# madronalabs/madronalib

Hardware: AMD Instinct MI355X
Metric: voice-samples/sec (SawGen->SVF chain) (higher is better)
Workload: dtype f32

## Files before the change

### madronalib_amd/csrc/mldsp_kernels.hpp

```cpp
#pragma once
#include "mlgpu_device_args.hpp"
#include "mldsp_procs.hpp"

namespace mldev
{
typedef float f32x4 __attribute__((ext_vector_type(4)));

constexpr int kChainBlock = 256;

constexpr int kMixStrip = 64 * 20 + 3 * 16 + 16;
template <int LO, int N>
struct MixTree16
{
  static __device__ __forceinline__ float sum(const float* col) { return MixTree16<LO, N / 2>::sum(col) + MixTree16<LO + N / 2, N / 2>::sum(col); }
};
template <int LO>
struct MixTree16<LO, 1>
{
  static __device__ __forceinline__ float sum(const float* col) { return col[LO * 20]; }
};

__device__ __forceinline__ void mix64_park(float* strip, int qq, f32x4 y)
{
  const uint32_t lane = threadIdx.x & 63u;
  *(f32x4*)(strip + lane * 20 + (lane >> 4) * 16 + 4 * qq) = y;
}
__device__ __forceinline__ void mix64_sum_store(const float* strip, float* row16)
{
  const uint32_t lane = threadIdx.x & 63u;
  __builtin_amdgcn_fence(__ATOMIC_RELEASE, "wavefront");
  __builtin_amdgcn_wave_barrier();
  __builtin_amdgcn_fence(__ATOMIC_ACQUIRE, "wavefront");
  const uint32_t s = lane & 15u, g = lane >> 4;
  const float t16 = MixTree16<0, 16>::sum(strip + g * (16 * 20 + 16) + s);
  const float t32 = t16 + u2f((uint32_t)__builtin_amdgcn_ds_bpermute((int)(((lane + 16u) & 63u) * 4u), (int)f2u(t16)));
  const float t64 = t32 + u2f((uint32_t)__builtin_amdgcn_ds_bpermute((int)(((lane + 32u) & 63u) * 4u), (int)f2u(t32)));
  if (lane < 16) row16[s] = t64;
  __builtin_amdgcn_wave_barrier();
}

template <bool MIX>
struct MixStrips
{
  static __device__ __forceinline__ float* mine() { return nullptr; }
};
template <>
struct MixStrips<true>
{
  static __device__ __forceinline__ float* mine()
  {
    __shared__ __attribute__((aligned(16))) float lds[(256 / 64) * kMixStrip];
    return lds + (threadIdx.x >> 6) * kMixStrip;
  }
};

constexpr int kHeadGeneral = 0, kHeadFast = 1, kHeadTrip = 2;
constexpr int kHeadTripSamples = 8;

template <class CH, bool HAS_SIGNAL, int HEAD, bool MIX = false, bool SCALED = false, bool LISTED = false>
__device__ __forceinline__ void run_voice(CH& ch, const ChainArgs& a, size_t v, float xc, float* strip = nullptr, bool live = true, size_t vs = 0,
                                          uint32_t* peak = nullptr)
{
  static_assert(HEAD != kHeadTrip || (!HAS_SIGNAL && CH::kHeadHasTrip), "trips want a launch-constant input and a head that has them");
  const size_t vin = LISTED ? vs : v;
  uint32_t pk = 0;
  const float mixGain = (SCALED && a.mixGains) ? a.mixGains[vin] : 1.f;
  const f32x4* pin = HAS_SIGNAL ? (const f32x4*)a.in.base + vin * a.in.strideV : nullptr;
  f32x4* pout = MIX ? nullptr : (f32x4*)a.out.base + v * a.out.strideV;
  const size_t inQ = a.in.strideQ, outQ = a.out.strideQ;
  const uint32_t slot = wave_slot();
  for (size_t t = 0; t < a.T; ++t)
  {
    const f32x4* pi = HAS_SIGNAL ? pin + t * a.in.strideT : nullptr;
    f32x4* po = MIX ? nullptr : pout + t * a.out.strideT;
    float s[kHeadTripSamples];
#pragma unroll 4
    for (int q = 0; q < 16; ++q)
    {
      if ((q & 3) == 0) take_turns_by_clock(slot, kTurnClockShift);
      f32x4 y;
      if constexpr (HEAD == kHeadTrip)
      {
        static_assert(kHeadTripSamples == 8, "a trip is two quads");
        if ((q & 1) == 0) ch.template next_head_trip<kHeadTripSamples>(xc, s);
        y = (q & 1) ? f32x4{s[4], s[5], s[6], s[7]} : f32x4{s[0], s[1], s[2], s[3]};
      }
      else
      {
        f32x4 x = {xc, xc, xc, xc};
        if constexpr (HAS_SIGNAL) x = __builtin_nontemporal_load(pi + q * inQ);
        y.x = ch.template next_head<HEAD == kHeadFast>(x.x);
        y.y = ch.template next_head<HEAD == kHeadFast>(x.y);
        y.z = ch.template next_head<HEAD == kHeadFast>(x.z);
        y.w = ch.template next_head<HEAD == kHeadFast>(x.w);
      }
      if constexpr (LISTED)
      {
        const uint32_t m0 = f2u(y.x) & 0x7fffffffu, m1 = f2u(y.y) & 0x7fffffffu, m2 = f2u(y.z) & 0x7fffffffu, m3 = f2u(y.w) & 0x7fffffffu;
        const uint32_t m01 = m0 > m1 ? m0 : m1, m23 = m2 > m3 ? m2 : m3, m = m01 > m23 ? m01 : m23;
        pk = pk > m ? pk : m;
      }
      if constexpr (MIX)
      {
        if constexpr (SCALED)
        {
          if (a.mixGains)
          {
            y.x *= mixGain;
            y.y *= mixGain;
            y.z *= mixGain;
            y.w *= mixGain;
          }
          if (!live) y = f32x4{0.f, 0.f, 0.f, 0.f};
        }
        mix64_park(strip, q & 3, y);
        if ((q & 3) == 3) mix64_sum_store(strip, a.mix + ((v >> 6) * a.T + t) * 64 + (size_t)(q & ~3) * 4);
      }
      else
        __builtin_nontemporal_store(y, po + q * outQ);
    }
    ch.end_vector();
  }
  if constexpr (LISTED) *peak = pk;
}

template <class CH, bool HAS_SIGNAL, bool MIX, bool SCALED, bool LISTED>
__device__ __forceinline__ void run_voice_as(int head, CH& ch, const ChainArgs& a, size_t v, float xc, float* strip, bool live, size_t vs, uint32_t* peak)
{
  if constexpr (!HAS_SIGNAL && CH::kHeadHasTrip)
  {
    if (head == kHeadTrip)
    {
      run_voice<CH, HAS_SIGNAL, kHeadTrip, MIX, SCALED, LISTED>(ch, a, v, xc, strip, live, vs, peak);
      return;
    }
  }
  if (head != kHeadGeneral)
    run_voice<CH, HAS_SIGNAL, kHeadFast, MIX, SCALED, LISTED>(ch, a, v, xc, strip, live, vs, peak);
  else
    run_voice<CH, HAS_SIGNAL, kHeadGeneral, MIX, SCALED, LISTED>(ch, a, v, xc, strip, live, vs, peak);
}

template <int OUT_G>
struct GroupStrips
{
  static __device__ __forceinline__ float* mine() { return nullptr; }
};
template <>
struct GroupStrips<16>
{
  static __device__ __forceinline__ float* mine()
  {
    __shared__ __attribute__((aligned(16))) float lds[(256 / 64) * kGroup16Strip];
    return lds + (threadIdx.x >> 6) * kGroup16Strip;
  }
};

template <class CH, bool HAS_SIGNAL, bool FAST_HEAD, int OUT_G, bool GAINS>
__device__ __forceinline__ void run_voice_groups(CH& ch, const ChainArgs& a, size_t v, float xc, float* strip)
{
  static_assert(OUT_G == 1 || OUT_G == 2 || OUT_G == 4 || OUT_G == 8 || OUT_G == 16, "group_sum_in_order's sizes, or none");
  const float gain = GAINS ? a.mixGains[v] : 1.f;
  const f32x4* pin = HAS_SIGNAL ? (const f32x4*)a.in.base + (v >> a.inGroupShift) * a.in.strideV : nullptr;
  f32x4* pout = (f32x4*)a.out.base + (v / OUT_G) * a.out.strideV;
  const bool lastOfGroup = (threadIdx.x & (OUT_G - 1)) == OUT_G - 1;
  const size_t inQ = a.in.strideQ, outQ = a.out.strideQ;
  const uint32_t slot = wave_slot();
  for (size_t t = 0; t < a.T; ++t)
  {
    const f32x4* pi = HAS_SIGNAL ? pin + t * a.in.strideT : nullptr;
    f32x4* po = pout + t * a.out.strideT;
#pragma unroll 4
    for (int q = 0; q < 16; ++q)
    {
      if ((q & 3) == 0) take_turns_by_clock(slot, kTurnClockShift);
      f32x4 x = {xc, xc, xc, xc};
      if constexpr (HAS_SIGNAL) x = __builtin_nontemporal_load(pi + q * inQ);
      f32x4 y;
      y.x = ch.template next_head<FAST_HEAD>(x.x);
      y.y = ch.template next_head<FAST_HEAD>(x.y);
      y.z = ch.template next_head<FAST_HEAD>(x.z);
      y.w = ch.template next_head<FAST_HEAD>(x.w);
      if constexpr (GAINS)
      {
        y.x *= gain;
        y.y *= gain;
        y.z *= gain;
        y.w *= gain;
      }
      if constexpr (OUT_G == 1)
        __builtin_nontemporal_store(y, po + q * outQ);
      else if constexpr (OUT_G == 16)
      {
        group16_park(strip, q & 3, y);
        if ((q & 3) == 3) group16_sum_store(strip, po + (size_t)(q - 3) * outQ, outQ);
      }
      else
      {
        y.x = group_sum_in_order<OUT_G>(y.x);
        y.y = group_sum_in_order<OUT_G>(y.y);
        y.z = group_sum_in_order<OUT_G>(y.z);
        y.w = group_sum_in_order<OUT_G>(y.w);
        if (lastOfGroup) __builtin_nontemporal_store(y, po + q * outQ);
      }
    }
    ch.end_vector();
  }
}

template <class CH, bool HAS_SIGNAL, bool MIX = false, int OUT_G = 0, bool LISTED = false>
__device__ __forceinline__ void chain_kernel_body(const ChainArgs& a)
{
  static_assert(!(MIX && OUT_G), "one summing form at a time");
  static_assert(!(LISTED && OUT_G), "no group form of a voice list");
  apply_fp_mode(a.flags);
  __shared__ float ldsTable[CH::kHasImpulse ? 32 : 1];
  float* const strip = OUT_G ? GroupStrips<OUT_G>::mine() : MixStrips<MIX>::mine();
  if constexpr (CH::kHasImpulse)
  {
    if (threadIdx.x < Proc<MLGPU_PROC_IMPULSE_GEN>::kTableSize) ldsTable[threadIdx.x] = a.impulseTable[threadIdx.x];
    __syncthreads();
  }
  size_t blk = blockIdx.x;
  const size_t nbFull = (size_t)gridDim.x & ~(size_t)7;
  if (blk < nbFull) blk = (blk & 7) * (nbFull >> 3) + (blk >> 3);
  size_t v = blk * kChainBlock + threadIdx.x;
  bool live = true;
  if constexpr (MIX)
  {
    if ((v & ~(size_t)63) >= a.V) return;
    live = v < a.V;
    if (!live) v = a.V - 1;
  }
  else if (v >= a.V)
    return;

  size_t vs = v, stride = a.V;
  if constexpr (LISTED)
  {
    vs = a.voiceList[v];
    stride = a.tableStride;
  }
  uint32_t pk = 0;

  CH ch;
  const VoiceMem mem{a.coeffs + vs, a.state + vs, stride};
  const KernelTables tables{ldsTable};
  ch.load(mem, tables);

  const float xc = (!HAS_SIGNAL && a.inConst) ? a.inConst[vs] : 0.f;

  bool fastHead = false;
  if constexpr (!HAS_SIGNAL && CH::kHeadHasFastPath) fastHead = (__builtin_amdgcn_ballot_w64(CH::head_input_is_odd(xc)) == 0);
  int head = fastHead ? kHeadFast : kHeadGeneral;
  if constexpr (!HAS_SIGNAL && CH::kHeadHasTrip)
  {
    if (fastHead && __builtin_amdgcn_ballot_w64(trip_freq_is_dense(xc, kHeadTripSamples)) == 0) head = kHeadTrip;
  }
  if constexpr (OUT_G != 0)
  {
    if (a.mixGains != nullptr)
    {
      if (fastHead)
        run_voice_groups<CH, HAS_SIGNAL, true, OUT_G, true>(ch, a, v, xc, strip);
      else
        run_voice_groups<CH, HAS_SIGNAL, false, OUT_G, true>(ch, a, v, xc, strip);
    }
    else if (fastHead)
      run_voice_groups<CH, HAS_SIGNAL, true, OUT_G, false>(ch, a, v, xc, strip);
    else
      run_voice_groups<CH, HAS_SIGNAL, false, OUT_G, false>(ch, a, v, xc, strip);
  }
  else if constexpr (MIX)
  {
    const bool scaled = a.mixGains != nullptr || __builtin_amdgcn_ballot_w64(!live) != 0;
    if (scaled)
      run_voice_as<CH, HAS_SIGNAL, true, true, LISTED>(head, ch, a, v, xc, strip, live, vs, &pk);
    else
      run_voice_as<CH, HAS_SIGNAL, true, false, LISTED>(head, ch, a, v, xc, strip, live, vs, &pk);
  }
  else
    run_voice_as<CH, HAS_SIGNAL, false, false, LISTED>(head, ch, a, v, xc, strip, live, vs, &pk);
  ch.store(mem);
  if constexpr (LISTED)
  {
    if (a.peaks != nullptr)
    {
      if (live) a.peaks[v] = pk;
    }
  }
}

template <class CH, bool HAS_SIGNAL>
__global__ __launch_bounds__(kChainBlock) void chain_kernel(const ChainArgs a)
{
  chain_kernel_body<CH, HAS_SIGNAL>(a);
}

template <class CH, bool HAS_SIGNAL>
__global__ __launch_bounds__(kChainBlock) void chain_mix_kernel(const ChainArgs a)
{
  chain_kernel_body<CH, HAS_SIGNAL, true>(a);
}

template <class CH, bool HAS_SIGNAL>
__global__ __launch_bounds__(kChainBlock) void chain_listed_kernel(const ChainArgs a)
{
  chain_kernel_body<CH, HAS_SIGNAL, false, 0, true>(a);
}
template <class CH, bool HAS_SIGNAL>
__global__ __launch_bounds__(kChainBlock) void chain_listed_mix_kernel(const ChainArgs a)
{
  chain_kernel_body<CH, HAS_SIGNAL, true, 0, true>(a);
}

template <class CH, bool HAS_SIGNAL, int OUT_G>
__global__ __launch_bounds__(kChainBlock) void chain_group_kernel(const ChainArgs a)
{
  chain_kernel_body<CH, HAS_SIGNAL, false, OUT_G>(a);
}

typedef float f32x2 __attribute__((ext_vector_type(2)));

template <int KIND, int N>
struct SvfCascade
{
  static_assert(N % 2 == 0, "stages are evaluated in pairs");
  static constexpr int NCK = (KIND == MLGPU_PROC_HIPASS) ? 4 : 3;
  static constexpr int NC = NCK * N, NS = 2 * N;
  static constexpr int H = N / 2;
  f32x2 g0[H], g1[H], g2[H], kk[H], ic1[H], ic2[H], r[H];

  template <class ARR>
  static MLD void put(ARR& arr, int s, float value)
  {
    if (s < H)
      arr[s].x = value;
    else
      arr[s - H].y = value;
  }
  template <class ARR>
  static MLD float get(const ARR& arr, int s) { return s < H ? arr[s].x : arr[s - H].y; }

  MLD void load(const VoiceMem& m)
  {
#pragma unroll
    for (int s = 0; s < N; ++s)
    {
      put(g0, s, m.c(NCK * s));
      put(g1, s, m.c(NCK * s + 1));
      put(g2, s, m.c(NCK * s + 2));
      put(kk, s, (KIND == MLGPU_PROC_HIPASS) ? m.c(NCK * s + 3) : 0.f);
      put(ic1, s, u2f(m.s(2 * s)));
      put(ic2, s, u2f(m.s(2 * s + 1)));
      put(r, s, 0.f);
    }
  }
  MLD void store(const VoiceMem& m) const
  {
#pragma unroll
    for (int s = 0; s < N; ++s)
    {
      m.set(2 * s, f2u(get(ic1, s)));
      m.set(2 * s + 1, f2u(get(ic2, s)));
    }
  }
  MLD float tick(float x) { return tick_in0(f32x2{x, r[H - 1].x}); }
  MLD float tick_in0(f32x2 in0) { return tick_common<false>(in0, in0); }
  MLD float tick_t0(f32x2 t00)
  {
    static_assert(KIND != MLGPU_PROC_HIPASS, "Hipass reads its input twice");
    return tick_common<true>(t00, t00);
  }
  template <bool HAVE_T0>
  MLD float tick_common(f32x2 in0, f32x2 t00)
  {
    f32x2 in[H], t0[H], a[H], b[H], c[H], d[H], t1[H], t2[H], v1[H], v2[H];
    const f32x2 two = {2.0f, 2.0f};
    in[0] = in0;
#pragma unroll
    for (int p = 1; p < H; ++p) in[p] = r[p - 1];
#pragma unroll
    for (int p = 0; p < H; ++p) t0[p] = in[p] - ic2[p];
    if constexpr (HAVE_T0) t0[0] = t00;
#pragma unroll
    for (int p = 0; p < H; ++p) b[p] = g1[p] * ic1[p];
#pragma unroll
    for (int p = 0; p < H; ++p) d[p] = g0[p] * ic1[p];
#pragma unroll
    for (int p = 0; p < H; ++p) a[p] = g0[p] * t0[p];
#pragma unroll
    for (int p = 0; p < H; ++p) c[p] = g2[p] * t0[p];
#pragma unroll
    for (int p = 0; p < H; ++p) t1[p] = a[p] + b[p];
#pragma unroll
    for (int p = 0; p < H; ++p) t2[p] = c[p] + d[p];
    if (KIND == MLGPU_PROC_LOPASS)
    {
#pragma unroll
      for (int p = 0; p < H; ++p) r[p] = t2[p] + ic2[p];
    }
    else if (KIND == MLGPU_PROC_BANDPASS)
    {
#pragma unroll
      for (int p = 0; p < H; ++p) r[p] = t1[p] + ic1[p];
    }
    else
    {
#pragma unroll
      for (int p = 0; p < H; ++p) v1[p] = t1[p] + ic1[p];
#pragma unroll
      for (int p = 0; p < H; ++p) v2[p] = t2[p] + ic2[p];
#pragma unroll
      for (int p = 0; p < H; ++p) v1[p] = kk[p] * v1[p];
#pragma unroll
      for (int p = 0; p < H; ++p) v1[p] = in[p] - v1[p];
#pragma unroll
      for (int p = 0; p < H; ++p) r[p] = v1[p] - v2[p];
    }
#pragma unroll
    for (int p = 0; p < H; ++p) ic1[p] = MLGPU_SVF_STRICT ? ic1[p] + two * t1[p] : __builtin_elementwise_fma(two, t1[p], ic1[p]);
#pragma unroll
    for (int p = 0; p < H; ++p) ic2[p] = MLGPU_SVF_STRICT ? ic2[p] + two * t2[p] : __builtin_elementwise_fma(two, t2[p], ic2[p]);
    return r[H - 1].y;
  }
  MLD float tick_masked(float x, int sLo, int sHi)
  {
    float in[N];
    in[0] = x;
#pragma unroll
    for (int s = 1; s < N; ++s) in[s] = get(r, s - 1);
#pragma unroll
    for (int s = 0; s < N; ++s)
    {
      if (s >= sLo && s <= sHi)
      {
        const float i1 = get(ic1, s), i2 = get(ic2, s);
        const float t0 = in[s] - i2;
        const float t1 = get(g0, s) * t0 + get(g1, s) * i1;
        const float t2 = get(g2, s) * t0 + get(g0, s) * i1;
        if (KIND == MLGPU_PROC_LOPASS)
          put(r, s, t2 + i2);
        else if (KIND == MLGPU_PROC_BANDPASS)
          put(r, s, t1 + i1);
        else
          put(r, s, in[s] - get(kk, s) * (t1 + i1) - (t2 + i2));
        put(ic1, s, svf_acc(i1, t1));
        put(ic2, s, svf_acc(i2, t2));
      }
    }
    return get(r, N - 1);
  }
};

template <class HEAD, int KIND, int N, bool HAS_SIGNAL>
__global__ __launch_bounds__(kChainBlock) void cascade_kernel(const ChainArgs a)
{
  static_assert(!HEAD::kHasImpulse, "ImpulseGen heads are not supported by the cascade kernel");
  static_assert((N - 1) % 4 != 0, "cascade lengths with (N - 1) % 4 == 0 need a bounded prefetch");
  apply_fp_mode(a.flags);
  size_t blk = blockIdx.x;
  const size_t nbFull = (size_t)gridDim.x & ~(size_t)7;
  if (blk < nbFull) blk = (blk & 7) * (nbFull >> 3) + (blk >> 3);
  const size_t v = blk * kChainBlock + threadIdx.x;
  if (v >= a.V) return;

  HEAD head;
  SvfCascade<KIND, N> c;
  const VoiceMem mh{a.coeffs + v, a.state + v, a.V};
  const VoiceMem mc{a.coeffs + (size_t)HEAD::NC * a.V + v, a.state + (size_t)HEAD::NS * a.V + v, a.V};
  const KernelTables tables{nullptr};
  head.load(mh, tables);
  c.load(mc);
  const float xc = (!HAS_SIGNAL && a.inConst) ? a.inConst[v] : 0.f;

  constexpr int D = N - 1;
  constexpr int A = D / 4, B = D % 4;
  const size_t S = a.T * 64;
  const f32x4* pin = HAS_SIGNAL ? (const f32x4*)a.in.base + v * a.in.strideV : nullptr;
  f32x4* pout = (f32x4*)a.out.base + v * a.out.strideV;
  auto inQuad = [&](size_t qi) { return pin + (qi >> 4) * a.in.strideT + (qi & 15) * a.in.strideQ; };
  auto outQuad = [&](size_t qi) { return pout + (qi >> 4) * a.out.strideT + (qi & 15) * a.out.strideQ; };
  auto inAt = [&](size_t i) -> float {
    if constexpr (HAS_SIGNAL) return ((const float*)inQuad(i >> 2))[i & 3];
    return xc;
  };

  for (int i = 0; i < D; ++i) c.tick_masked(head.next(inAt((size_t)i)), 0, i);

  constexpr int QT = 4;
  const size_t Q = (S - D) / 4;
  size_t q = 0;
  if constexpr (HAS_SIGNAL)
  {
    f32x4 w[QT + 1];
    if (Q >= QT)
    {
#pragma unroll
      for (int k = 0; k < QT + 1; ++k) w[k] = __builtin_nontemporal_load(inQuad((size_t)(A + k)));
    }
    for (; q + QT <= Q; q += QT)
    {
      const bool more = (q + 2 * QT <= Q);
      f32x4 nx[QT];
      if (more)
      {
#pragma unroll
        for (int k = 0; k < QT; ++k) nx[k] = __builtin_nontemporal_load(inQuad(q + A + QT + 1 + k));
      }
#pragma unroll
      for (int g = 0; g < QT; ++g)
      {
        f32x4 y;
#pragma unroll
        for (int j = 0; j < 4; ++j)
        {
          const int e = B + j;
          const float x = (e < 4) ? w[g][e & 3] : w[g + 1][e & 3];
          y[j] = c.tick(head.next(x));
        }
        __builtin_nontemporal_store(y, outQuad(q + g));
      }
      if (more)
      {
        w[0] = w[QT];
#pragma unroll
        for (int k = 0; k < QT; ++k) w[k + 1] = nx[k];
      }
    }
  }
  else
  {
    for (; q + 4 <= Q; q += 4)
    {
#pragma unroll
      for (int g = 0; g < 4; ++g)
      {
        f32x4 y;
#pragma unroll
        for (int j = 0; j < 4; ++j) y[j] = c.tick(head.next(xc));
        __builtin_nontemporal_store(y, outQuad(q + g));
      }
    }
  }
  for (size_t i = D + 4 * q; i < S + D; ++i)
  {
    float x = 0.f;
    if (i < S) x = head.next(inAt(i));
    const int sLo = (i < S) ? 0 : (int)(i - S + 1);
    const float y = c.tick_masked(x, sLo, N - 1);
    const size_t n = i - D;
    ((float*)outQuad(n >> 2))[n & 3] = y;
  }
  head.store(mh);
  c.store(mc);
}

template <int LPC>
struct LaneGroup
{
// ... 150 lines not shown
```

### madronalib_amd/csrc/mldsp_procs.hpp

```cpp
#pragma once
#include "mldsp_math.hpp"
#ifdef __HIPCC_RTC__
#include "mlgpu.h"
#else
#include "../../include/mlgpu.h"
#endif

namespace mldev
{
struct VoiceMem
{
  const float* coeffs;
  uint32_t* state;
  size_t V;
  float* mem{nullptr};
  uint32_t memMask{0};
  MLD float* ringPtr(int ringIdx, uint32_t i) const
  {
    if (addr32) return (float*)((char*)(mem + (size_t)((uint32_t)ringIdx * (memMask + 1)) * V) + (__umul24(i, V4) + lane4));
    return mem + (size_t)((uint32_t)ringIdx * (memMask + 1) + i) * V;
  }
  MLD float ring(int ringIdx, uint32_t i) const { return *ringPtr(ringIdx, i); }
  MLD void ringSet(int ringIdx, uint32_t i, float x) const { *ringPtr(ringIdx, i) = x; }
  float* lds{nullptr};
  uint32_t ldsHist{0};
  uint32_t lane4{0}, V4{0};
  bool addr32{false};
  MLD float c(int i) const { return coeffs[(size_t)i * V]; }
  MLD uint32_t s(int i) const { return state[(size_t)i * V]; }
  MLD void set(int i, uint32_t x) const { state[(size_t)i * V] = x; }
};

struct KernelTables
{
  const float* impulse_table;
};

constexpr float kStepsPerCycle = 4294967296.0f;
constexpr float kCyclesPerStep = 2.3283064365386963e-10f;

constexpr uint32_t kSqrt2Bits = 0x3fb50505u;
constexpr uint32_t kSineDomainBits = 0x40b50505u;
constexpr uint32_t kSineScaleBits = 0x3f87c3b6u;
constexpr uint32_t kSineFlipBits = 0x40350505u;
constexpr uint32_t kOneSixthBits = 0x3e2aaaabu;

MLD float phasor_next(uint32_t& omega32, float cyclesPerSample)
{
  const float steps = cyclesPerSample * kStepsPerCycle;
  const int32_t istep = sse_cvt(steps);
  omega32 += (uint32_t)istep;
  const float hi = (float)(int32_t)(omega32 >> 1);
  return hi * 4.656612873077392578125e-10f;
}

constexpr float kPhaseUnit = 4.656612873077392578125e-10f;
constexpr float kPhaseScale = 2147483648.0f;
MLD float phasor_next_hi(uint32_t& omega32, float cyclesPerSample)
{
  const float steps = cyclesPerSample * kStepsPerCycle;
  const int32_t istep = sse_cvt(steps);
  omega32 += (uint32_t)istep;
  asm("" : "+v"(omega32));
  return (float)(int32_t)(omega32 >> 1);
}

MLD float div_nr(float n, float d)
{
  const float r0 = __builtin_amdgcn_rcpf(d);
  const float e = __builtin_fmaf(-d, r0, 1.0f);
  const float r1 = __builtin_fmaf(e, r0, r0);
  const float q0 = n * r1;
  const float rem0 = __builtin_fmaf(-d, q0, n);
  const float q1 = __builtin_fmaf(rem0, r1, q0);
  const float rem1 = __builtin_fmaf(-d, q1, n);
  return __builtin_fmaf(rem1, r1, q1);
}

MLD bool blep_freq_is_odd(float dt) { return (dt > 0.f) && !((dt >= 0x1p-64f) && (dt <= 0x1p+64f)); }

MLD bool blep_freq_not_regular(float dt) { return (f2u(dt) - 0x1F800000u) > (0x5F800000u - 0x1F800000u); }

template <bool FAST>
struct BlepFreq
{
  float dt, omdt;
  bool otherOdd;
  static MLD BlepFreq make(float dt, bool otherwiseOdd = false)
  {
    BlepFreq f;
    f.dt = dt;
    f.omdt = 1.0f - dt;
    f.otherOdd = otherwiseOdd;
    return f;
  }
  MLD bool lo(float t) const { return t < dt; }
  MLD bool hi(float t) const { return t > omdt; }
  MLD bool anyLaneOdd() const { return __builtin_amdgcn_ballot_w64((!FAST && blep_freq_not_regular(dt)) || otherOdd) != 0; }
  MLD float correction(float t, bool isLo, bool full) const
  {
    const float num = isLo ? t : (t - 1.0f);
    float q;
    if (full)
      q = num / dt;
    else
      q = div_nr(num, dt);
    const float qq = q * q;
    const float twoq_qq = full ? ((q + q) - qq) : __builtin_fmaf(2.0f, q, -qq);
    const float clo = twoq_qq - 1.0f;
    const float chi = ((qq + q) + q) + 1.0f;
    return isLo ? clo : chi;
  }
};

template <bool SKIP, bool FAST>
MLD float poly_blep(float t, const BlepFreq<FAST>& f)
{
  const bool lo = f.lo(t), hi = f.hi(t);
  if (SKIP && __builtin_amdgcn_ballot_w64(lo || hi) == 0) return 0.f;
  const float c = f.correction(t, lo, f.anyLaneOdd());
  return (lo || hi) ? c : 0.f;
}
template <bool FAST, bool SKIP = false>
MLD float poly_blep(float t, float dt)
{
  return poly_blep<SKIP>(t, BlepFreq<FAST>::make(dt));
}

MLD bool phase_is_odd(float p) { return !(((p >= 0x1p-31f) && (p <= 1.0f)) || (p == 0.f)); }

template <bool FAST, bool SKIP = false, bool ANY_PHASE = false>
MLD float phasor_to_saw(float p, float cps)
{
  const float saw = ANY_PHASE ? (p * 2.f - 1.f) : __builtin_fmaf(p, 2.f, -1.f);
  return saw - poly_blep<SKIP>(p, BlepFreq<FAST>::make(cps, ANY_PHASE && phase_is_odd(p)));
}

MLD bool pulse_width_is_odd(float w) { return !(w >= 0.f && w <= 1.0f); }

template <bool FAST, bool SKIP = false, bool ANY_PHASE = false, bool REGULAR_W = false>
MLD float phasor_to_pulse(float p, float cps, float w)
{
  const float pulse = (p >= w) ? -1.f : 1.f;
  const float d = p - w + 1.0f;
  const float down = REGULAR_W ? __builtin_amdgcn_fractf(d) : d - (float)sse_cvtt(d);
  const bool downOdd = ANY_PHASE ? phase_is_odd(down) : (!REGULAR_W && !(abs_ps(down) <= 2.0f));
  const BlepFreq<FAST> f = BlepFreq<FAST>::make(cps, (ANY_PHASE && phase_is_odd(p)) || downOdd);
  const bool loUp = f.lo(p), nearUp = loUp || f.hi(p);
  const bool loDown = f.lo(down), nearDown = loDown || f.hi(down);
  if (SKIP && __builtin_amdgcn_ballot_w64(nearUp || nearDown) == 0) return pulse;
  const bool full = f.anyLaneOdd();
  if (!(ANY_PHASE && full) && __builtin_amdgcn_ballot_w64(nearUp && nearDown) == 0)
  {
    const float c = f.correction(nearDown ? down : p, nearDown ? loDown : loUp, full);
    return nearDown ? (pulse - c) : (nearUp ? (pulse + c) : pulse);
  }
  const float cUp = f.correction(p, loUp, full), cDown = f.correction(down, loDown, full);
  return (pulse + (nearUp ? cUp : 0.f)) - (nearDown ? cDown : 0.f);
}

constexpr float kTripMaxFreq(int n) { return 0.5f / (float)n; }
constexpr float kTripTiny = 0x1p-22f, kTripNearOne = 1.0f - 0x1p-22f;
constexpr float kTripTinyShifted = 0x1p-21f, kTripNearOneShifted = 1.0f - 0x1p-21f;
MLD bool trip_freq_is_dense(float dt, int n) { return !(dt > 0.f && dt <= kTripMaxFreq(n)); }
MLD uint32_t trip_umin(uint32_t a, uint32_t b) { return a < b ? a : b; }
MLD uint32_t trip_umax(uint32_t a, uint32_t b) { return a > b ? a : b; }

MLD float phasor_to_sine(float p)
{
  const float sqrt2 = u2f(kSqrt2Bits);
  const float omega = p * u2f(kSineDomainBits) + (-sqrt2);
  const float tri = (omega > sqrt2) ? (u2f(kSineFlipBits) - omega) : omega;
  return (u2f(kSineScaleBits) * tri) * (1.0f - (tri * tri) * u2f(kOneSixthBits));
}

MLD float phasor_hi_to_sine(float hi)
{
  const float sqrt2 = u2f(kSqrt2Bits);
  const float omega = hi * u2f(kSineDomainBits - (31u << 23)) + (-sqrt2);
  const float refl = u2f(kSineFlipBits) - omega;
  float tri;
  asm("v_min_f32 %0, %1, %2" : "=v"(tri) : "v"(omega), "v"(refl));
  return (u2f(kSineScaleBits) * tri) * (1.0f - (tri * tri) * u2f(kOneSixthBits));
}

template <int KIND>
struct Proc;


template <>
struct Proc<MLGPU_PROC_PHASOR_GEN>
{
  static constexpr int NC = 0, NS = 1;
  uint32_t omega32;
  MLD void load(const VoiceMem& m, const KernelTables&) { omega32 = m.s(0); }
  MLD void store(const VoiceMem& m) const { m.set(0, omega32); }
  MLD float next(float cps) { return phasor_next(omega32, cps); }
  MLD void end_vector() {}
};

template <>
struct Proc<MLGPU_PROC_SINE_GEN>
{
  static constexpr int NC = 0, NS = 1;
  uint32_t omega32;
  MLD void load(const VoiceMem& m, const KernelTables&) { omega32 = m.s(0); }
  MLD void store(const VoiceMem& m) const { m.set(0, omega32); }
  MLD float next(float cps) { return phasor_hi_to_sine(phasor_next_hi(omega32, cps)); }
  MLD void end_vector() {}
};

template <>
struct Proc<MLGPU_PROC_TEST_SINE_GEN>
{
  static constexpr int NC = 0, NS = 1;
  float omega;
  MLD void load(const VoiceMem& m, const KernelTables&) { omega = u2f(m.s(0)); }
  MLD void store(const VoiceMem& m) const { m.set(0, f2u(omega)); }
  MLD float next(float cps)
  {
    const float twoPi = 6.2831853071795864769252867f;
    const float step = twoPi * cps;
    omega += step;
    if (omega > twoPi) omega -= twoPi;
    return libm_sinf(omega);
  }
  MLD void end_vector() {}
};

template <>
struct Proc<MLGPU_PROC_SAW_GEN>
{
  static constexpr int NC = 0, NS = 1;
  uint32_t omega32;
  MLD void load(const VoiceMem& m, const KernelTables&) { omega32 = m.s(0); }
  MLD void store(const VoiceMem& m) const { m.set(0, omega32); }
  template <bool FAST, bool SKIP = false>
  MLD float step(float cps)
  {
    return phasor_to_saw<FAST, SKIP>(phasor_next(omega32, cps), cps);
  }
  MLD float next(float cps) { return step<false, true>(cps); }
  MLD float next_fast(float cps) { return step<true>(cps); }
  MLD float next_u(float cps, bool odd) { return odd ? step<false>(cps) : step<true>(cps); }
  static MLD bool input_is_odd(float cps) { return blep_freq_is_odd(cps); }
  template <int N>
  MLD void trip_u(float cps, bool odd, bool dense, float (&out)[N])
  {
    if (!dense)
    {
      const BlepFreq<true> f = BlepFreq<true>::make(cps);
      const float dtS = f.dt * kPhaseScale, omdtS = f.omdt * kPhaseScale;
      const uint32_t before = omega32;
      float h[N];
      uint32_t lo = 0u, hi = 0u;
#pragma unroll
      for (int i = 0; i < N; ++i)
      {
        h[i] = phasor_next_hi(omega32, cps);
        lo = i ? trip_umin(lo, f2u(h[i])) : f2u(h[i]);
        hi = i ? trip_umax(hi, f2u(h[i])) : f2u(h[i]);
      }
      if (__builtin_amdgcn_ballot_w64(u2f(lo) < kTripTiny * kPhaseScale || u2f(hi) > kTripNearOne * kPhaseScale) == 0)
      {
        const float cLo = f.correction(u2f(lo) * kPhaseUnit, true, false), cHi = f.correction(u2f(hi) * kPhaseUnit, false, false);
#pragma unroll
        for (int i = 0; i < N; ++i)
        {
          const float saw = __builtin_fmaf(h[i], 2.f * kPhaseUnit, -1.f);
          out[i] = saw - ((h[i] < dtS) ? cLo : ((h[i] > omdtS) ? cHi : 0.f));
        }
        return;
      }
      omega32 = before;
    }
#pragma unroll
    for (int i = 0; i < N; ++i) out[i] = next_u(cps, odd);
  }
  MLD void end_vector() {}
};

template <>
struct Proc<MLGPU_PROC_PULSE_GEN>
{
  static constexpr int NC = 1, NS = 1;
  uint32_t omega32;
  float width;
  MLD void load(const VoiceMem& m, const KernelTables&)
  {
    width = m.c(0);
    omega32 = m.s(0);
  }
  MLD void store(const VoiceMem& m) const { m.set(0, omega32); }
  template <bool FAST, bool SKIP = false, bool REGULAR_W = false>
  MLD float step(float cps, float w)
  {
    return phasor_to_pulse<FAST, SKIP, false, REGULAR_W>(phasor_next(omega32, cps), cps, w);
  }
  MLD float next(float cps) { return step<false, true>(cps, width); }
  MLD float next_fast(float cps) { return step<true>(cps, width); }
  MLD float next2(float cps, float w) { return step<false, true>(cps, w); }
  MLD float next_u(float cps, bool odd) { return odd ? step<false>(cps, width) : step<true, false, true>(cps, width); }
  MLD float next_u(float cps, float w, bool odd) { return odd ? step<false>(cps, w) : step<true, false, true>(cps, w); }
  MLD float next_uw(float cps, float w, bool odd) { return odd ? step<false>(cps, w) : step<true>(cps, w); }
  MLD float next_sw(float cps, bool oddW) { return oddW ? step<false, true>(cps, width) : step<false, true, true>(cps, width); }
  MLD float next_sw(float cps, float w, bool oddW) { return oddW ? step<false, true>(cps, w) : step<false, true, true>(cps, w); }
  static MLD bool input_is_odd(float cps) { return blep_freq_is_odd(cps); }
  template <int N>
  MLD void trip_u(float cps, float w, bool odd, bool dense, float (&out)[N])
  {
    if (!dense)
    {
      const BlepFreq<true> f = BlepFreq<true>::make(cps);
      const float dtS = f.dt * kPhaseScale, omdtS = f.omdt * kPhaseScale, wS = w * kPhaseScale;
      const uint32_t before = omega32;
      float h[N], d[N];
      uint32_t lo = 0u, hi = 0u, dlo = 0u, dhi = 0u;
#pragma unroll
      for (int i = 0; i < N; ++i)
      {
        h[i] = phasor_next_hi(omega32, cps);
        d[i] = __builtin_amdgcn_fractf(__builtin_fmaf(h[i], kPhaseUnit, -w) + 1.0f);
        lo = i ? trip_umin(lo, f2u(h[i])) : f2u(h[i]);
        hi = i ? trip_umax(hi, f2u(h[i])) : f2u(h[i]);
        dlo = i ? trip_umin(dlo, f2u(d[i])) : f2u(d[i]);
        dhi = i ? trip_umax(dhi, f2u(d[i])) : f2u(d[i]);
      }
      const bool suspect = u2f(lo) < kTripTiny * kPhaseScale || u2f(hi) > kTripNearOne * kPhaseScale || u2f(dlo) < kTripTinyShifted || u2f(dhi) > kTripNearOneShifted;
      if (__builtin_amdgcn_ballot_w64(suspect) == 0)
      {
        const float cUpLo = f.correction(u2f(lo) * kPhaseUnit, true, false), cUpHi = f.correction(u2f(hi) * kPhaseUnit, false, false);
        const float cDownLo = f.correction(u2f(dlo), true, false), cDownHi = f.correction(u2f(dhi), false, false);
#pragma unroll
        for (int i = 0; i < N; ++i)
        {
          const float pulse = (h[i] >= wS) ? -1.f : 1.f;
          const float cUp = (h[i] < dtS) ? cUpLo : ((h[i] > omdtS) ? cUpHi : 0.f);
          const float cDown = f.lo(d[i]) ? cDownLo : (f.hi(d[i]) ? cDownHi : 0.f);
          out[i] = (pulse + cUp) - cDown;
        }
        return;
      }
      omega32 = before;
    }
#pragma unroll
    for (int i = 0; i < N; ++i) out[i] = next_u(cps, w, odd);
  }
  template <int N>
  MLD void trip_u(float cps, bool odd, bool dense, float (&out)[N])
  {
    trip_u<N>(cps, width, odd, dense, out);
  }
  MLD void end_vector() {}
};

template <>
struct Proc<MLGPU_PROC_NOISE_GEN>
{
  static constexpr int NC = 0, NS = 1;
  uint32_t seed;
  MLD void load(const VoiceMem& m, const KernelTables&) { seed = m.s(0); }
  MLD void store(const VoiceMem& m) const { m.set(0, seed); }
  MLD float next(float)
  {
    seed = seed * 0x0019660Du + 0x3C6EF35Fu;
    const uint32_t temp = ((seed >> 9) & 0x007FFFFFu) | 0x3F800000u;
    return __builtin_fmaf(u2f(temp), 2.f, -3.f);
  }
  MLD void end_vector() {}
};

template <>
struct Proc<MLGPU_PROC_TICK_GEN>
{
  static constexpr int NC = 0, NS = 1;
  float omega;
  MLD void load(const VoiceMem& m, const KernelTables&) { omega = u2f(m.s(0)); }
  MLD void store(const VoiceMem& m) const { m.set(0, f2u(omega)); }
  MLD float next(float cps)
  {
    float y = 0.f;
    omega += cps;
    if (omega > 1.0f)
    {
      omega -= 1.0f;
      y = 1.0f;
    }
    return y;
  }
  MLD void end_vector() {}
};

template <>
struct Proc<MLGPU_PROC_IMPULSE_GEN>
{
  static constexpr int NC = 0, NS = 2;
  static constexpr int kTableSize = 17;
  float omega;
  int32_t counter;
  const float* table;
  MLD void load(const VoiceMem& m, const KernelTables& t)
  {
    omega = u2f(m.s(0));
    counter = (int32_t)m.s(1);
    table = t.impulse_table;
  }
  MLD void store(const VoiceMem& m) const
  {
    m.set(0, f2u(omega));
    m.set(1, (uint32_t)counter);
  }
  MLD float next(float cps)
  {
    float y = 0.f;
    omega += cps;
    if (omega > 1.0f)
    {
      omega -= 1.0f;
      counter = 0;
    }
    if (counter < kTableSize)
    {
      y = table[counter];
      counter++;
    }
    return y;
  }
  MLD void end_vector() {}
};

template <>
struct Proc<MLGPU_PROC_ONE_SHOT_GEN>
{
  static constexpr int NC = 0, NS = 3;
  uint32_t omega32, gate, prev;
  MLD void load(const VoiceMem& m, const KernelTables&)
  {
    omega32 = m.s(0);
    gate = m.s(1);
    prev = m.s(2);
  }
  MLD void store(const VoiceMem& m) const
  {
    m.set(0, omega32);
    m.set(1, gate);
    m.set(2, prev);
  }
  MLD float next(float cps)
  {
    const float steps = cps * kStepsPerCycle;
    const int32_t istep = sse_cvt(steps);
    omega32 += (uint32_t)istep * gate;
    if (omega32 < prev)
    {
      gate = 0;
      omega32 = 0;
    }
    prev = omega32;
    return uint_to_float(omega32) * kCyclesPerStep;
  }
  MLD void end_vector() {}
};


#ifndef MLGPU_SVF_STRICT
#define MLGPU_SVF_STRICT 0
#endif
MLD float svf_acc(float ic, float t)
{
#if MLGPU_SVF_STRICT
  return ic + 2.0f * t;
#else
  return __builtin_fmaf(2.0f, t, ic);
#endif
}
MLD float svf_flip(float v, float ic)
{
#if MLGPU_SVF_STRICT
  return 2.0f * v - ic;
#else
  return __builtin_fmaf(2.0f, v, -ic);
#endif
}

template <int KIND>
struct SvfCore
{
  static constexpr int NC = (KIND == MLGPU_PROC_HIPASS) ? 4 : 3;
  static constexpr int NS = 2;
  float g0, g1, g2, k;
  float ic1eq, ic2eq;
  MLD void load(const VoiceMem& m, const KernelTables&)
  {
    g0 = m.c(0);
    g1 = m.c(1);
    g2 = m.c(2);
    k = (KIND == MLGPU_PROC_HIPASS) ? m.c(3) : 0.f;
    ic1eq = u2f(m.s(0));
    ic2eq = u2f(m.s(1));
  }
  MLD void store(const VoiceMem& m) const
  {
    m.set(0, f2u(ic1eq));
    m.set(1, f2u(ic2eq));
  }
  MLD float next(float v0)
  {
    const float t0 = v0 - ic2eq;
    const float t1 = g0 * t0 + g1 * ic1eq;
    const float t2 = g2 * t0 + g0 * ic1eq;
    float y;
    if (KIND == MLGPU_PROC_LOPASS)
    {
      y = t2 + ic2eq;
    }
    else if (KIND == MLGPU_PROC_BANDPASS)
    {
      y = t1 + ic1eq;
    }
    else
    {
      const float v1 = t1 + ic1eq;
      const float v2 = t2 + ic2eq;
      y = v0 - k * v1 - v2;
    }
    ic1eq = svf_acc(ic1eq, t1);
    ic2eq = svf_acc(ic2eq, t2);
    return y;
  }
  MLD void end_vector() {}
};
template <>
struct Proc<MLGPU_PROC_LOPASS> : SvfCore<MLGPU_PROC_LOPASS>
{
  MLD float next(float v0, float omega, float kq)
  {
    omega = sse_min_bound(omega, 0.5f);
    kq = sse_max_bound(kq, 0.01f);
    const float piOmega = 3.1415926535897932384626433832795f * omega;
    const float twoPiOmega = 2.0f * piOmega;
    const bool regularK = (kq <= 1.98f);
    const uint32_t kOut = regularK ? 0u : 0x80000000u;
    const bool q0 = (((f2u(twoPiOmega) - f2u(2.f * kSinfMin))) | kOut) < (f2u(kSinfT1) - f2u(2.f * kSinfMin));
    float s1, s2, nrm;
    if (__builtin_expect(__builtin_amdgcn_ballot_w64(!q0) == 0, 1))
    {
      s1 = libm_sinf_q0(piOmega);
      s2 = libm_sinf_q0(twoPiOmega);
      nrm = div_nr(1.0f, 2.f + kq * s2);
    }
    else if (__builtin_amdgcn_ballot_w64(!((piOmega >= kSinfMin) && regularK)) == 0)
    {
      libm_sinf_pair(piOmega, twoPiOmega, s1, s2);
      nrm = div_nr(1.0f, 2.f + kq * s2);
    }
    else
    {
      float s[2];
#pragma unroll 1
      for (int i = 0; i < 2; ++i) s[i] = libm_sinf(i ? twoPiOmega : piOmega);
      s1 = s[0];
      s2 = s[1];
      nrm = 1.0f / (2.f + kq * s2);
    }
    const float c0 = s2 * nrm;
    const float c1 = (-2.f * s1 * s1 - kq * s2) * nrm;
    const float c2 = (2.0f * s1 * s1) * nrm;
    const float t0 = v0 - ic2eq;
    const float t1 = c0 * t0 + c1 * ic1eq;
    const float t2 = c2 * t0 + c0 * ic1eq;
    const float y = t2 + ic2eq;
    ic1eq = svf_acc(ic1eq, t1);
    ic2eq = svf_acc(ic2eq, t2);
    return y;
  }
  using SvfCore<MLGPU_PROC_LOPASS>::next;
};
template <>
struct Proc<MLGPU_PROC_HIPASS> : SvfCore<MLGPU_PROC_HIPASS>
{
// ... 1419 lines not shown
    const float va = pathA(xe);
    const float vb = pathB(xo);
    const float y = (va + b1) * 0.5f;
    b1 = vb;
    return y;
  }
};

template <>
struct Proc<MLGPU_PROC_HALF_BAND>
{
  static constexpr int NC = 0, NS = 9;
  HalfBandCore hb;
  MLD void load(const VoiceMem& m, const KernelTables&) { hb.load(m); }
  MLD void store(const VoiceMem& m) const { hb.store(m); }
  MLD float up_a(float x) { return hb.pathA(x); }
  MLD float up_b(float x) { return hb.pathB(x); }
  MLD float down(float xe, float xo) { return hb.down(xe, xo); }
  MLD void end_vector() {}
};

template <>
struct Proc<MLGPU_PROC_HALF_BAND_BUFFERED>
{
  static constexpr int NC = 0, NS = 9 + MLGPU_FLOATS_PER_DSPVECTOR;
  HalfBandCore hb;
  VoiceMem mem;
  MLD void load(const VoiceMem& m, const KernelTables&)
  {
    mem = m;
    hb.load(m);
  }
  MLD void store(const VoiceMem& m) const { hb.store(m); }
  float cur[4];
  MLD void begin_quad(int q)
  {
#pragma unroll
    for (int k = 0; k < 4; ++k) cur[k] = u2f(mem.s(9 + 4 * q + k));
  }
  MLD float delayed(int n) const { return cur[n & 3]; }
  MLD float delayedAt(int m) const { return u2f(mem.s(9 + m)); }
  MLD void push(int n, float x)
  {
    const float ya = hb.pathA(x);
    const float yb = hb.pathB(x);
    mem.set(9 + n - 1, f2u(ya));
    mem.set(9 + n, f2u(yb));
  }
  MLD void end_vector() {}
};

template <>
struct Proc<MLGPU_PROC_TEMPO_LOCK>
{
  static constexpr int NC = 0, NS = 2;
  float omega, x1v, dydt;
  bool stopped;
  MLD void load(const VoiceMem& m, const KernelTables&)
  {
    omega = u2f(m.s(0));
    x1v = u2f(m.s(1));
    dydt = 0.f;
    stopped = false;
  }
  MLD void store(const VoiceMem& m) const
  {
    m.set(0, f2u(omega));
    m.set(1, f2u(x1v));
  }
  MLD void begin_vector(float x0, float x1, float dydx, float isr)
  {
    stopped = (x0 == -1.0f);
    if (stopped)
    {
      omega = -1.0f;
      return;
    }
    float dxdt;
    if (omega > -1.f)
    {
      float dx = x0 - x1v;
      if (dx < 0.f) dx += 1.f;
      dxdt = dx / 64.f;
      dydt = dxdt * dydx;
      x1v = x0;
    }
    else
    {
      dxdt = x1 - x0;
      dydt = dxdt * dydx;
      x1v = x0 - dxdt * 64.f;
      omega = __builtin_fmodf(x0 * dydx, 1.0f);
    }
    bool lock = false;
    if (abs_ps(dydx - __builtin_roundf(dydx)) < 0.001f) lock = true;
    const float rdydx = 1.0f / dydx;
    if (abs_ps(rdydx - __builtin_roundf(rdydx)) < 0.001f) lock = true;
    if (lock)
    {
      float error;
      if (dydx >= 1.f)
      {
        const float ref = x0 * dydx;
        error = omega - (ref - __builtin_floorf(ref));
      }
      else
      {
        const float ref = omega / dydx;
        error = (ref - __builtin_floorf(ref)) - x0;
      }
      const float errorDiff = __builtin_roundf(error) - error;
      float correction = errorDiff * isr * 4.0f;
      const float lo = -dydt * 0.5f, hi = dydt * 1.0f;
      correction = (correction < lo) ? lo : (correction > hi ? hi : correction);
      dydt += correction;
    }
  }
  MLD float next_n(int)
  {
    if (stopped) return 0.f;
    const float y = omega;
    omega += dydt;
    if (omega > 1.0f) omega -= 1.0f;
    return y;
  }
  float x0h;
  bool starting;
  MLD float next_x(int n, float x, float dydx, float isr)
  {
    if (n == 0)
    {
      x0h = x;
      starting = !(x == -1.0f) && !(omega > -1.f);
      if (starting)
      {
        stopped = false;
        return __builtin_fmodf(x * dydx, 1.0f);
      }
      begin_vector(x, 0.f, dydx, isr);
    }
    else if (n == 1 && starting)
    {
      begin_vector(x0h, x, dydx, isr);
      omega += dydt;
      if (omega > 1.0f) omega -= 1.0f;
    }
    return next_n(n);
  }
  MLD void end_vector() {}
};


template <int N>
MLD bool trip_locked(Proc<MLGPU_PROC_SAW_GEN>& saw, Proc<MLGPU_PROC_PULSE_GEN>& pulse, float cps, float w, float (&outSaw)[N], float (&outPulse)[N])
{
  {
    const BlepFreq<true> f = BlepFreq<true>::make(cps);
    const float dtS = f.dt * kPhaseScale, omdtS = f.omdt * kPhaseScale, wS = w * kPhaseScale;
    uint32_t omega32 = saw.omega32;
    float h[N], d[N];
    uint32_t lo = 0u, hi = 0u, dlo = 0u, dhi = 0u;
#pragma unroll
    for (int i = 0; i < N; ++i)
    {
      h[i] = phasor_next_hi(omega32, cps);
      d[i] = __builtin_amdgcn_fractf(__builtin_fmaf(h[i], kPhaseUnit, -w) + 1.0f);
      lo = i ? trip_umin(lo, f2u(h[i])) : f2u(h[i]);
      hi = i ? trip_umax(hi, f2u(h[i])) : f2u(h[i]);
      dlo = i ? trip_umin(dlo, f2u(d[i])) : f2u(d[i]);
      dhi = i ? trip_umax(dhi, f2u(d[i])) : f2u(d[i]);
    }
    const bool suspect = u2f(lo) < kTripTiny * kPhaseScale || u2f(hi) > kTripNearOne * kPhaseScale || u2f(dlo) < kTripTinyShifted || u2f(dhi) > kTripNearOneShifted;
    if (__builtin_amdgcn_ballot_w64(suspect) == 0)
    {
      const float cLo = f.correction(u2f(lo) * kPhaseUnit, true, false), cHi = f.correction(u2f(hi) * kPhaseUnit, false, false);
      const float cDownLo = f.correction(u2f(dlo), true, false), cDownHi = f.correction(u2f(dhi), false, false);
#pragma unroll
      for (int i = 0; i < N; ++i)
      {
        const float cUp = (h[i] < dtS) ? cLo : ((h[i] > omdtS) ? cHi : 0.f);
        const float cDown = f.lo(d[i]) ? cDownLo : (f.hi(d[i]) ? cDownHi : 0.f);
        outSaw[i] = __builtin_fmaf(h[i], 2.f * kPhaseUnit, -1.f) - cUp;
        outPulse[i] = (((h[i] >= wS) ? -1.f : 1.f) + cUp) - cDown;
      }
      saw.omega32 = omega32;
      pulse.omega32 = omega32;
      return true;
    }
  }
  return false;
}

template <bool REGULAR_W>
MLD void step_locked_stream(Proc<MLGPU_PROC_SAW_GEN>& saw, Proc<MLGPU_PROC_PULSE_GEN>& pulse, float cps, float w, float& outSaw, float& outPulse)
{
  const float p = phasor_next(saw.omega32, cps);
  pulse.omega32 = saw.omega32;
  const float sawv = __builtin_fmaf(p, 2.f, -1.f);
  const float pulsev = (p >= w) ? -1.f : 1.f;
  const float d = p - w + 1.0f;
  const float down = REGULAR_W ? __builtin_amdgcn_fractf(d) : d - (float)sse_cvtt(d);
  const bool downOdd = !REGULAR_W && !(abs_ps(down) <= 2.0f);
  const BlepFreq<false> f = BlepFreq<false>::make(cps, downOdd);
  const bool loUp = f.lo(p), nearUp = loUp || f.hi(p);
  const bool loDown = f.lo(down), nearDown = loDown || f.hi(down);
  outSaw = sawv;
  outPulse = pulsev;
  if (__builtin_amdgcn_ballot_w64(nearUp || nearDown) == 0) return;
  const bool full = f.anyLaneOdd();
  if (__builtin_amdgcn_ballot_w64(nearUp && nearDown) == 0)
  {
    const float c = f.correction(nearDown ? down : p, nearDown ? loDown : loUp, full);
    outPulse = nearDown ? (pulsev - c) : (nearUp ? (pulsev + c) : pulsev);
    outSaw = nearUp ? (sawv - c) : sawv;
    return;
  }
  const float cUp = f.correction(p, loUp, full), cDown = f.correction(down, loDown, full);
  outPulse = (pulsev + (nearUp ? cUp : 0.f)) - (nearDown ? cDown : 0.f);
  outSaw = sawv - (nearUp ? cUp : 0.f);
}

template <class P, class = void>
struct HasFastPath
{
  static constexpr bool value = false;
};
template <class P>
struct HasFastPath<P, decltype((void)&P::input_is_odd)>
{
  static constexpr bool value = true;
};

template <int... KINDS>
struct Chain;

template <>
struct Chain<>
{
  static constexpr int NC = 0, NS = 0;
  static constexpr bool kHasImpulse = false;
  MLD void load(VoiceMem, const KernelTables&) {}
  MLD void store(VoiceMem) const {}
  MLD float next(float x) { return x; }
  MLD void end_vector() {}
  static constexpr bool kHeadHasFastPath = false;
  static constexpr bool kHeadHasTrip = false;
  static MLD bool head_input_is_odd(float) { return false; }
  template <bool FAST>
  MLD float next_head(float x)
  {
    return x;
  }
};

template <int K0, int... KS>
struct Chain<K0, KS...>
{
  Proc<K0> head;
  Chain<KS...> tail;
  static constexpr int NC = Proc<K0>::NC + Chain<KS...>::NC;
  static constexpr int NS = Proc<K0>::NS + Chain<KS...>::NS;
  static constexpr bool kHasImpulse = (K0 == MLGPU_PROC_IMPULSE_GEN) || Chain<KS...>::kHasImpulse;
  MLD void load(VoiceMem m, const KernelTables& t)
  {
    head.load(m, t);
    m.coeffs += (size_t)Proc<K0>::NC * m.V;
    m.state += (size_t)Proc<K0>::NS * m.V;
    tail.load(m, t);
  }
  MLD void store(VoiceMem m) const
  {
    head.store(m);
    m.coeffs += (size_t)Proc<K0>::NC * m.V;
    m.state += (size_t)Proc<K0>::NS * m.V;
    tail.store(m);
  }
  MLD float next(float x) { return tail.next(head.next(x)); }
  static constexpr bool kHeadHasFastPath = HasFastPath<Proc<K0>>::value;
  static MLD bool head_input_is_odd(float x)
  {
    if constexpr (kHeadHasFastPath)
      return Proc<K0>::input_is_odd(x);
    else
      return false;
  }
  template <bool FAST>
  MLD float next_head(float x)
  {
    if constexpr (FAST && kHeadHasFastPath)
      return tail.next(head.next_fast(x));
    else
      return tail.next(head.next(x));
  }
  static constexpr bool kHeadHasTrip = kHeadHasFastPath && (K0 == MLGPU_PROC_SAW_GEN);
  template <int N>
  MLD void next_head_trip(float x, float (&y)[N])
  {
    static_assert(kHeadHasTrip, "a head with a trip form");
    float s[N];
    head.template trip_u<N>(x,  false,  false, s);
#pragma unroll
    for (int i = 0; i < N; ++i) y[i] = tail.next(s[i]);
  }
  MLD void end_vector()
  {
    head.end_vector();
    tail.end_vector();
  }
};

}
```

Baseline: 1415 billion.

## Add 16-sample saw trip head software-pipelined with SVF tail

Adds a kHeadTrip16 path for the SawGen head. It computes 16 phasor samples per trip with a single ballot-checked BLEP correction, where the existing trip covers 8. The loop is software-pipelined so that the next trip's phase computation is interleaved with the filter tail processing the previous trip's samples, using sched barriers and asm register pins to force the interleave. The path is chosen when every lane's frequency is low enough for 16-sample trips and no output groups are used. In exchange it raises register pressure, and the slow fallback is a serial per-sample recompute with dynamic array selects.

```diff
diff --git a/madronalib_amd/csrc/mldsp_kernels.hpp b/madronalib_amd/csrc/mldsp_kernels.hpp
--- a/madronalib_amd/csrc/mldsp_kernels.hpp
+++ b/madronalib_amd/csrc/mldsp_kernels.hpp
@@ -54,14 +54,14 @@
   }
 };
 
-constexpr int kHeadGeneral = 0, kHeadFast = 1, kHeadTrip = 2;
+constexpr int kHeadGeneral = 0, kHeadFast = 1, kHeadTrip = 2, kHeadTrip16 = 3;
 constexpr int kHeadTripSamples = 8;
 
 template <class CH, bool HAS_SIGNAL, int HEAD, bool MIX = false, bool SCALED = false, bool LISTED = false>
 __device__ __forceinline__ void run_voice(CH& ch, const ChainArgs& a, size_t v, float xc, float* strip = nullptr, bool live = true, size_t vs = 0,
                                           uint32_t* peak = nullptr)
 {
-  static_assert(HEAD != kHeadTrip || (!HAS_SIGNAL && CH::kHeadHasTrip), "trips want a launch-constant input and a head that has them");
+  static_assert((HEAD != kHeadTrip && HEAD != kHeadTrip16) || (!HAS_SIGNAL && CH::kHeadHasTrip), "trips want a launch-constant input and a head that has them");
   const size_t vin = LISTED ? vs : v;
   uint32_t pk = 0;
   const float mixGain = (SCALED && a.mixGains) ? a.mixGains[vin] : 1.f;
@@ -69,36 +69,22 @@
   f32x4* pout = MIX ? nullptr : (f32x4*)a.out.base + v * a.out.strideV;
   const size_t inQ = a.in.strideQ, outQ = a.out.strideQ;
   const uint32_t slot = wave_slot();
-  for (size_t t = 0; t < a.T; ++t)
-  {
-    const f32x4* pi = HAS_SIGNAL ? pin + t * a.in.strideT : nullptr;
-    f32x4* po = MIX ? nullptr : pout + t * a.out.strideT;
-    float s[kHeadTripSamples];
-#pragma unroll 4
-    for (int q = 0; q < 16; ++q)
-    {
-      if ((q & 3) == 0) take_turns_by_clock(slot, kTurnClockShift);
-      f32x4 y;
-      if constexpr (HEAD == kHeadTrip)
-      {
-        static_assert(kHeadTripSamples == 8, "a trip is two quads");
-        if ((q & 1) == 0) ch.template next_head_trip<kHeadTripSamples>(xc, s);
-        y = (q & 1) ? f32x4{s[4], s[5], s[6], s[7]} : f32x4{s[0], s[1], s[2], s[3]};
-      }
-      else
-      {
-        f32x4 x = {xc, xc, xc, xc};
-        if constexpr (HAS_SIGNAL) x = __builtin_nontemporal_load(pi + q * inQ);
-        y.x = ch.template next_head<HEAD == kHeadFast>(x.x);
-        y.y = ch.template next_head<HEAD == kHeadFast>(x.y);
-        y.z = ch.template next_head<HEAD == kHeadFast>(x.z);
-        y.w = ch.template next_head<HEAD == kHeadFast>(x.w);
-      }
+  if constexpr (HEAD == kHeadTrip16)
+  {
+    if (a.T == 0) return;
+    Trip16Phases trip;
+    float s[16];
+    uint32_t pk16 = 0;
+    f32x4 y;
+    auto tail_sample = [&](size_t t, int r, int i, float x) {
+      y[i & 3] = ch.tail_next(x);
+      if ((i & 3) != 3) return;
+      const int q = 4 * r + (i >> 2);
       if constexpr (LISTED)
       {
         const uint32_t m0 = f2u(y.x) & 0x7fffffffu, m1 = f2u(y.y) & 0x7fffffffu, m2 = f2u(y.z) & 0x7fffffffu, m3 = f2u(y.w) & 0x7fffffffu;
         const uint32_t m01 = m0 > m1 ? m0 : m1, m23 = m2 > m3 ? m2 : m3, m = m01 > m23 ? m01 : m23;
-        pk = pk > m ? pk : m;
+        pk16 = pk16 > m ? pk16 : m;
       }
       if constexpr (MIX)
       {
@@ -117,6 +103,88 @@
         if ((q & 3) == 3) mix64_sum_store(strip, a.mix + ((v >> 6) * a.T + t) * 64 + (size_t)(q & ~3) * 4);
       }
       else
+        __builtin_nontemporal_store(y, pout + t * a.out.strideT + q * outQ);
+    };
+    ch.head_trip16_begin(trip);
+#pragma unroll
+    for (int i = 0; i < 16; ++i) ch.head_trip16_phase(xc, trip, i);
+    ch.head_trip16_samples(xc, trip, s);
+    const size_t lastTrip = 4 * a.T - 1;
+    for (size_t k = 0; k < lastTrip; ++k)
+    {
+      const size_t t = k >> 2;
+      const int r = (int)(k & 3);
+      take_turns_by_clock(slot, kTurnClockShift);
+      ch.head_trip16_begin(trip);
+#pragma unroll
+      for (int i = 0; i < 16; ++i)
+      {
+        ch.head_trip16_phase(xc, trip, i);
+        tail_sample(t, r, i, s[i]);
+        if (i & 1)
+        {
+          asm volatile("" : "+v"(trip.lo), "+v"(trip.hi));
+          __builtin_amdgcn_sched_barrier(0);
+        }
+      }
+      if (r == 3) ch.end_vector();
+      ch.head_trip16_samples(xc, trip, s);
+    }
+    take_turns_by_clock(slot, kTurnClockShift);
+#pragma unroll
+    for (int i = 0; i < 16; ++i) tail_sample(a.T - 1, 3, i, s[i]);
+    ch.end_vector();
+    if constexpr (LISTED) *peak = pk16;
+    return;
+  }
+  for (size_t t = 0; t < a.T; ++t)
+  {
+    const f32x4* pi = HAS_SIGNAL ? pin + t * a.in.strideT : nullptr;
+    f32x4* po = MIX ? nullptr : pout + t * a.out.strideT;
+    float s[kHeadTripSamples];
+#pragma unroll 4
+    for (int q = 0; q < 16; ++q)
+    {
+      if ((q & 3) == 0) take_turns_by_clock(slot, kTurnClockShift);
+      f32x4 y;
+      if constexpr (HEAD == kHeadTrip)
+      {
+        static_assert(kHeadTripSamples == 8, "a trip is two quads");
+        if ((q & 1) == 0) ch.template next_head_trip<kHeadTripSamples>(xc, s);
+        y = (q & 1) ? f32x4{s[4], s[5], s[6], s[7]} : f32x4{s[0], s[1], s[2], s[3]};
+      }
+      else
+      {
+        f32x4 x = {xc, xc, xc, xc};
+        if constexpr (HAS_SIGNAL) x = __builtin_nontemporal_load(pi + q * inQ);
+        y.x = ch.template next_head<HEAD == kHeadFast>(x.x);
+        y.y = ch.template next_head<HEAD == kHeadFast>(x.y);
+        y.z = ch.template next_head<HEAD == kHeadFast>(x.z);
+        y.w = ch.template next_head<HEAD == kHeadFast>(x.w);
+      }
+      if constexpr (LISTED)
+      {
+        const uint32_t m0 = f2u(y.x) & 0x7fffffffu, m1 = f2u(y.y) & 0x7fffffffu, m2 = f2u(y.z) & 0x7fffffffu, m3 = f2u(y.w) & 0x7fffffffu;
+        const uint32_t m01 = m0 > m1 ? m0 : m1, m23 = m2 > m3 ? m2 : m3, m = m01 > m23 ? m01 : m23;
+        pk = pk > m ? pk : m;
+      }
+      if constexpr (MIX)
+      {
+        if constexpr (SCALED)
+        {
+          if (a.mixGains)
+          {
+            y.x *= mixGain;
+            y.y *= mixGain;
+            y.z *= mixGain;
+            y.w *= mixGain;
+          }
+          if (!live) y = f32x4{0.f, 0.f, 0.f, 0.f};
+        }
+        mix64_park(strip, q & 3, y);
+        if ((q & 3) == 3) mix64_sum_store(strip, a.mix + ((v >> 6) * a.T + t) * 64 + (size_t)(q & ~3) * 4);
+      }
+      else
         __builtin_nontemporal_store(y, po + q * outQ);
     }
     ch.end_vector();
@@ -129,6 +197,11 @@
 {
   if constexpr (!HAS_SIGNAL && CH::kHeadHasTrip)
   {
+    if (head == kHeadTrip16)
+    {
+      run_voice<CH, HAS_SIGNAL, kHeadTrip16, MIX, SCALED, LISTED>(ch, a, v, xc, strip, live, vs, peak);
+      return;
+    }
     if (head == kHeadTrip)
     {
       run_voice<CH, HAS_SIGNAL, kHeadTrip, MIX, SCALED, LISTED>(ch, a, v, xc, strip, live, vs, peak);
@@ -255,7 +328,8 @@
   int head = fastHead ? kHeadFast : kHeadGeneral;
   if constexpr (!HAS_SIGNAL && CH::kHeadHasTrip)
   {
-    if (fastHead && __builtin_amdgcn_ballot_w64(trip_freq_is_dense(xc, kHeadTripSamples)) == 0) head = kHeadTrip;
+    if (fastHead && __builtin_amdgcn_ballot_w64(trip_freq_is_dense(xc, kHeadTripSamples)) == 0)
+      head = (OUT_G == 0 && __builtin_amdgcn_ballot_w64(trip_freq_is_dense(xc, 16)) == 0) ? kHeadTrip16 : kHeadTrip;
   }
   if constexpr (OUT_G != 0)
   {
diff --git a/madronalib_amd/csrc/mldsp_procs.hpp b/madronalib_amd/csrc/mldsp_procs.hpp
--- a/madronalib_amd/csrc/mldsp_procs.hpp
+++ b/madronalib_amd/csrc/mldsp_procs.hpp
@@ -165,6 +165,12 @@
 MLD bool trip_freq_is_dense(float dt, int n) { return !(dt > 0.f && dt <= kTripMaxFreq(n)); }
 MLD uint32_t trip_umin(uint32_t a, uint32_t b) { return a < b ? a : b; }
 MLD uint32_t trip_umax(uint32_t a, uint32_t b) { return a > b ? a : b; }
+struct Trip16Phases
+{
+  float h[16];
+  uint32_t lo, hi;
+  uint32_t before;
+};
 
 MLD float phasor_to_sine(float p)
 {
@@ -276,6 +282,40 @@
     }
 #pragma unroll
     for (int i = 0; i < N; ++i) out[i] = next_u(cps, odd);
+  }
+  MLD void trip16_begin(Trip16Phases& t) const { t.before = omega32; }
+  MLD void trip16_phase(float cps, Trip16Phases& t, int i)
+  {
+    t.h[i] = phasor_next_hi(omega32, cps);
+    t.lo = i ? trip_umin(t.lo, f2u(t.h[i])) : f2u(t.h[i]);
+    t.hi = i ? trip_umax(t.hi, f2u(t.h[i])) : f2u(t.h[i]);
+  }
+  MLD void trip16_samples(float cps, const Trip16Phases& t, float (&out)[16]) const
+  {
+    const BlepFreq<true> f = BlepFreq<true>::make(cps);
+    const float dtS = f.dt * kPhaseScale, omdtS = f.omdt * kPhaseScale;
+    if (__builtin_amdgcn_ballot_w64(u2f(t.lo) < kTripTiny * kPhaseScale || u2f(t.hi) > kTripNearOne * kPhaseScale) == 0)
+    {
+      const float cLo = f.correction(u2f(t.lo) * kPhaseUnit, true, false), cHi = f.correction(u2f(t.hi) * kPhaseUnit, false, false);
+#pragma unroll
+      for (int i = 0; i < 16; ++i)
+      {
+        const float saw = __builtin_fmaf(t.h[i], 2.f * kPhaseUnit, -1.f);
+        out[i] = saw - ((t.h[i] < dtS) ? cLo : ((t.h[i] > omdtS) ? cHi : 0.f));
+      }
+      return;
+    }
+    Proc again;
+    again.omega32 = t.before;
+#pragma unroll
+    for (int k = 0; k < 16; ++k) out[k] = 0.f;
+#pragma unroll 1
+    for (int i = 0; i < 16; ++i)
+    {
+      const float y = again.next_u(cps,  false);
+#pragma unroll
+      for (int k = 0; k < 16; ++k) out[k] = (k == i) ? y : out[k];
+    }
   }
   MLD void end_vector() {}
 };
@@ -2301,6 +2341,10 @@
 #pragma unroll
     for (int i = 0; i < N; ++i) y[i] = tail.next(s[i]);
   }
+  MLD void head_trip16_begin(Trip16Phases& t) const { head.trip16_begin(t); }
+  MLD void head_trip16_phase(float x, Trip16Phases& t, int i) { head.trip16_phase(x, t, i); }
+  MLD void head_trip16_samples(float x, const Trip16Phases& t, float (&s)[16]) const { head.trip16_samples(x, t, s); }
+  MLD float tail_next(float s) { return tail.next(s); }
   MLD void end_vector()
   {
     head.end_vector();
```

After: 1469 billion (median of 4 runs). +3.8%, better.
